# RohitMovva/VexAutonomousPlanner

Measured on NVIDIA B200. Metric: profiled trajectories/sec (8-node paths), higher is better.
Workload: dtype f64

## Files before the change

vexautonomousplanner_b200/csrc/vap_device.cuh:

```cuda
#pragma once
#include <cstdint>
#include <math.h>

#define NA 12
enum { A_X = 0, A_Y, A_TURN, A_WAIT, A_MAXVEL, A_MAXACC, A_TX, A_TY, A_INMAG, A_OUTMAG, A_RCOS, A_RSIN };
#define F_REVERSE 1
#define F_STOP 2
#define F_TANGENT 4
#define APA 4
enum { P_T = 0, P_WAIT, P_MAXVEL, P_MAXACC };

#define ST_OK 0
#define ST_FALSE (-1)
#define ST_INDEX (-2)
#define ST_VALUE (-3)
#define ST_CAPACITY (-4)
#define ST_DIVERGED (-5)
#define ST_EVENTS (-6)
#define VAP_ROW_LIMIT 50000000LL

#define VAP_PI 3.141592653589793

__device__ __forceinline__ void cp_async16(void* smem, const void* gmem)
{
    unsigned sa = (unsigned)__cvta_generic_to_shared(smem);
    asm volatile("cp.async.ca.shared.global [%0], [%1], 16;" ::"r"(sa), "l"(gmem));
}
__device__ __forceinline__ void cp_async_commit() { asm volatile("cp.async.commit_group;" ::); }
template <int N>
__device__ __forceinline__ void cp_async_wait() { asm volatile("cp.async.wait_group %0;" ::"n"(N) : "memory"); }

__device__ __forceinline__ void mbar_init(unsigned a, unsigned count)
{
    asm volatile("mbarrier.init.shared::cta.b64 [%0], %1;" ::"r"(a), "r"(count) : "memory");
}
__device__ __forceinline__ void mbar_expect_tx(unsigned a, unsigned bytes)
{
    asm volatile("mbarrier.arrive.expect_tx.shared::cta.b64 _, [%0], %1;" ::"r"(a), "r"(bytes) : "memory");
}
__device__ __forceinline__ void bulk_g2s(unsigned dst, const void* src, unsigned bytes, unsigned mbar)
{
    asm volatile("cp.async.bulk.shared::cluster.global.mbarrier::complete_tx::bytes [%0], [%1], %2, [%3];"
                 ::"r"(dst), "l"(src), "r"(bytes), "r"(mbar) : "memory");
}
__device__ __forceinline__ void mbar_wait(unsigned a, unsigned parity)
{
    asm volatile("{\n"
                 ".reg .pred P1;\n"
                 "LAB_WAIT:\n"
                 "mbarrier.try_wait.parity.shared::cta.b64 P1, [%0], %1;\n"
                 "@P1 bra DONE;\n"
                 "bra LAB_WAIT;\n"
                 "DONE:\n"
                 "}" ::"r"(a), "r"(parity) : "memory");
}

__device__ __forceinline__ void fence_mbar_init() { asm volatile("fence.mbarrier_init.release.cluster;" ::: "memory"); }
__device__ __forceinline__ void fence_proxy_async() { asm volatile("fence.proxy.async.shared::cta;" ::: "memory"); }

#ifdef VAP_BOUNDS_CHECK
#define VAP_DIAG_SITES 32
__device__ unsigned long long g_vap_diag[VAP_DIAG_SITES];
#define VAP_CHECK(site, cond) do { if (!(cond)) atomicAdd(&g_vap_diag[site], 1ull); else atomicAdd(&g_vap_diag[16 + ((site) & 15)], 1ull); } while (0)
#else
#define VAP_CHECK(site, cond) do { } while (0)
#endif

struct PathTile { long long b; unsigned x; };
__device__ __forceinline__ PathTile path_tile(unsigned tiles_x)
{
    PathTile p;
    const unsigned q = blockIdx.x / tiles_x;
    p.b = q; p.x = blockIdx.x - q * tiles_x;
    return p;
}

__device__ __forceinline__ double pymin(double a, double b) { return (b < a) ? b : a; }
__device__ __forceinline__ double pymax(double a, double b) { return (b > a) ? b : a; }
__device__ __forceinline__ double norm1d(double x, double y) { return sqrt(fma(y, y, x * x)); }
__device__ __forceinline__ double norm_ax1(double x, double y) { return sqrt(x * x + y * y); }
__device__ __forceinline__ double frac1(double t) { return t - floor(t); }
__device__ __forceinline__ double pymod_pos(double x, double y)
{
    double m = fmod(x, y);
    if (m != 0.0) { if (m < 0) m += y; } else m = 0.0;
    return m;
}

template <int WHICH>
__device__ __forceinline__ void basis(double t, double* H)
{
    double t2 = t * t, t3 = t2 * t;
    if (WHICH == 0) {
        double t4 = t3 * t, t5 = t4 * t;
        H[0] = 1 - 10 * t3 + 15 * t4 - 6 * t5;
        H[1] = 10 * t3 - 15 * t4 + 6 * t5;
        H[2] = t - 6 * t3 + 8 * t4 - 3 * t5;
        H[3] = -4 * t3 + 7 * t4 - 3 * t5;
        H[4] = 0.5 * t2 - 1.5 * t3 + 1.5 * t4 - 0.5 * t5;
        H[5] = 0.5 * t3 - t4 + 0.5 * t5;
    } else if (WHICH == 1) {
        double t4 = t3 * t;
        H[0] = -30 * t2 + 60 * t3 - 30 * t4;
        H[1] = 30 * t2 - 60 * t3 + 30 * t4;
        H[2] = 1 - 18 * t2 + 32 * t3 - 15 * t4;
        H[3] = -12 * t2 + 28 * t3 - 15 * t4;
        H[4] = t - 4.5 * t2 + 6 * t3 - 2.5 * t4;
        H[5] = 1.5 * t2 - 4 * t3 + 2.5 * t4;
    } else {
        H[0] = -60 * t + 180 * t2 - 120 * t3;
        H[1] = 60 * t - 180 * t2 + 120 * t3;
        H[2] = -36 * t + 96 * t2 - 60 * t3;
        H[3] = -24 * t + 84 * t2 - 60 * t3;
        H[4] = 1 - 9 * t + 18 * t2 - 10 * t3;
        H[5] = 3 * t - 12 * t2 + 10 * t3;
    }
}

__device__ __forceinline__ void normalize_param(double t, int nseg, double pend, int& idx, double& u)
{
    double tt = pymax(0.0, pymin(t, pend));
    idx = (int)tt;
    if (idx == nseg) idx = nseg - 1;
    u = tt - (double)idx;
}

template <int WHICH>
__device__ __forceinline__ void eval_spline(const double* __restrict__ seg, int nseg, double pend, double t,
                                            double& ox, double& oy)
{
    int idx; double u;
    normalize_param(t, nseg, pend, idx, u);
    double H[6];
    basis<WHICH>(u, H);
    const double2* s = reinterpret_cast<const double2*>(seg + (size_t)idx * 12);
    double ax = 0.0, ay = 0.0;
#pragma unroll
    for (int i = 0; i < 6; i++) { double2 r = __ldg(s + i); ax += H[i] * r.x; ay += H[i] * r.y; }
    ox = ax; oy = ay;
}

__device__ __forceinline__ void eval_spline_d12(const double* __restrict__ seg, int nseg, double pend, double t,
                                                double& dx, double& dy, double& ddx, double& ddy)
{
    int idx; double u;
    normalize_param(t, nseg, pend, idx, u);
    double H1[6], H2[6];
    basis<1>(u, H1);
    basis<2>(u, H2);
    const double2* s = reinterpret_cast<const double2*>(seg + (size_t)idx * 12);
    double ax = 0.0, ay = 0.0, bx = 0.0, by = 0.0;
#pragma unroll
    for (int i = 0; i < 6; i++) {
        double2 r = __ldg(s + i);
        ax += H1[i] * r.x; ay += H1[i] * r.y;
        bx += H2[i] * r.x; by += H2[i] * r.y;
    }
    dx = ax; dy = ay; ddx = bx; ddy = by;
}

struct PathGeo {
    const double* seg;
    const int* first;
    const double* pend;
    int S;
};
__device__ __forceinline__ int map_spline(const PathGeo& g, double t)
{
    int k = 0;
    if (g.S <= 8) {
        while (k < g.S - 1 && !(t <= (double)g.first[k + 1])) k++;
    } else {
        int lo = 0, hi = g.S - 1;
        while (lo < hi) {
            int mid = (lo + hi) >> 1;
            if (t <= (double)g.first[mid + 1]) hi = mid; else lo = mid + 1;
        }
        k = lo;
    }
    return k;
}
__device__ __forceinline__ PathGeo path_geo(long long b, int N_max, const double* seg, const int* first_node,
                                            const double* param_end, const int* n_splines)
{
    PathGeo g;
    g.seg = seg + (size_t)b * (N_max - 1) * 12;
    g.first = first_node + (size_t)b * (N_max + 1);
    g.pend = param_end + (size_t)b * N_max;
    g.S = n_splines[b];
    return g;
}

template <int WHICH>
__device__ __forceinline__ void eval_path(const PathGeo& g, double t, double& ox, double& oy)
{
    int k = map_spline(g, t);
    int f0 = g.first[k], f1 = g.first[k + 1];
    eval_spline<WHICH>(g.seg + (size_t)f0 * 12, f1 - f0, g.pend[k], t - (double)f0, ox, oy);
}
__device__ __forceinline__ void eval_path_d12(const PathGeo& g, double t, double& dx, double& dy, double& ddx,
                                              double& ddy)
{
    int k = map_spline(g, t);
    int f0 = g.first[k], f1 = g.first[k + 1];
    eval_spline_d12(g.seg + (size_t)f0 * 12, f1 - f0, g.pend[k], t - (double)f0, dx, dy, ddx, ddy);
}

__device__ __forceinline__ void curv_heading(double dx, double dy, double ddx, double ddy, double& kap, double& th)
{
    double s2 = dx * dx + dy * dy;
    double num = dx * ddy - dy * ddx;
    kap = (s2 >= 1e-10) ? num / (s2 * sqrt(s2)) : 0.0;
    th = atan2(dy, dx);
}

__device__ __forceinline__ double prop_param(long long j, long long P, int n, double step)
{
    return (j == P - 1) ? (double)(n - 1) : (double)j * step;
}
__device__ __forceinline__ long long prop_lower_bound(double t, long long P, int n, double step, double inv_step)
{
    double e = t * inv_step;
    long long j = (e > 0.0) ? (e < (double)P ? (long long)e : P) : 0;
    while (j > 0 && prop_param(j - 1, P, n, step) >= t) j--;
    while (j < P && prop_param(j, P, n, step) < t) j++;
    return j;
}
__device__ __forceinline__ double snap_gather(const double* __restrict__ vals, double t, long long P, int n,
                                              double step, double inv_step)
{
    long long idx = prop_lower_bound(t, P, n, step, inv_step);
    if (idx == 0) return vals[0];
    if (idx >= P) return vals[P - 1];
    double t0 = prop_param(idx - 1, P, n, step), t1 = prop_param(idx, P, n, step);
    if (frac1(t0) != frac1(t1)) return (frac1(t) > 0.5) ? vals[idx - 1] : vals[idx];
    double v0 = vals[idx - 1], v1 = vals[idx];
    return v0 + (v1 - v0) * (t - t0) / (t1 - t0);
}
__device__ __forceinline__ void snap_gather2(const double* __restrict__ ka, const double* __restrict__ ha, double t,
                                             long long P, int n, double step, double inv_step, double& k, double& h)
{
    long long idx = prop_lower_bound(t, P, n, step, inv_step);
    if (idx == 0) { k = ka[0]; h = ha[0]; return; }
    if (idx >= P) { k = ka[P - 1]; h = ha[P - 1]; return; }
    double t0 = prop_param(idx - 1, P, n, step), t1 = prop_param(idx, P, n, step);
    if (frac1(t0) != frac1(t1)) {
        long long g = (frac1(t) > 0.5) ? idx - 1 : idx;
        k = ka[g]; h = ha[g];
        return;
    }
    double w = (t - t0);
    k = ka[idx - 1] + (ka[idx] - ka[idx - 1]) * w / (t1 - t0);
    h = ha[idx - 1] + (ha[idx] - ha[idx - 1]) * w / (t1 - t0);
}

__device__ __forceinline__ double distance_to_time(const double* __restrict__ ld, const double* __restrict__ lt,
                                                   long long Q, double total, int n, double d, long long& hint)
{
    if (d <= 0) return 0.0;
    if (d >= total) return (double)(n - 1);
    long long idx;
    long long h = hint;
    if (h >= 1 && h < Q && ld[h - 1] < d) {
        idx = h;
        int steps = 0;
        while (idx < Q && ld[idx] < d && steps < 4) { idx++; steps++; }
        if (!(idx < Q && ld[idx] >= d)) h = -1;
    } else h = -1;
    if (h < 0) {
        long long lo = 0, hi = Q;
        while (lo < hi) {
            long long mid = lo + ((hi - lo) >> 1);
            if (ld[mid] < d) lo = mid + 1; else hi = mid;
        }
        idx = lo;
    }
    hint = idx;
    if (idx == 0) return lt[0];
    double d0 = ld[idx - 1], d1 = ld[idx], t0 = lt[idx - 1], t1 = lt[idx];
    return t0 + (t1 - t0) * (d - d0) / (d1 - d0);
}

struct PropGrid {
    int P, n;
    double step, inv_step;
};
__device__ __forceinline__ PropGrid prop_grid(int spn, int n)
{
    PropGrid g;
    g.P = spn * n; g.n = n;
    g.step = (double)(n - 1) / (double)(g.P - 1);
    g.inv_step = 1.0 / g.step;
    return g;
}
__device__ __forceinline__ double prop_param32(int j, const PropGrid& g)
{
    return (j == g.P - 1) ? (double)(g.n - 1) : (double)j * g.step;
}
__device__ __forceinline__ void snap_gather2_32(const double* __restrict__ ka, const double* __restrict__ ha, double t,
                                                const PropGrid& g, double& k, double& h)
{
    double e = t * g.inv_step;
    int j = (e > 0.0) ? (e < (double)g.P ? __double2int_rz(e) : g.P) : 0;
    while (j > 0 && prop_param32(j - 1, g) >= t) j--;
    while (j < g.P && prop_param32(j, g) < t) j++;
    if (j == 0) { k = ka[0]; h = ha[0]; return; }
    if (j >= g.P) { k = ka[g.P - 1]; h = ha[g.P - 1]; return; }
    double t0 = prop_param32(j - 1, g), t1 = prop_param32(j, g);
    if (frac1(t0) != frac1(t1)) {
        int q = (frac1(t) > 0.5) ? j - 1 : j;
        k = ka[q]; h = ha[q];
// ... 108 lines not shown
```

vexautonomousplanner_b200/csrc/vap_kernels.cu:

```cuda
#include <cuda_runtime.h>
#include <cstdio>
#include <cstring>
#include <cstdlib>

#include "../../include/vap.h"
#include "vap_device.cuh"
#include "vap_velocity.cuh"
#include "vap_timeloop.cuh"
#include "vap_format.cuh"

static thread_local char g_err[512] = "";
static int set_err(const char* where, cudaError_t e)
{
    snprintf(g_err, sizeof(g_err), "%s: %s", where, cudaGetErrorString(e));
    return -100;
}
static int arg_err(const char* msg)
{
    snprintf(g_err, sizeof(g_err), "%s", msg);
    return -101;
}
#define CHECK_LAUNCH(name)                                   \
    do {                                                     \
        cudaError_t e__ = cudaGetLastError();                \
// ... 187 lines not shown
        int m = i - cur + 1;
        RunView R;
        R.px = na + (size_t)cur * NA + A_X; R.py = na + (size_t)cur * NA + A_Y; R.stride = NA;
        R.has = nf + cur; R.has_stride = 1; R.in_mask = F_TANGENT; R.out_mask = F_TANGENT;
        R.tin = tin + 2 * cur; R.tout = tout + 2 * cur;
        fit_run(m, R, use_start, usx, usy, have_end, etx, ety, sg + (size_t)cur * 12, sl + cur, pr ? pr + pc : nullptr,
                pe + S, scr, use_start, have_end, nullptr, dv ? dv + (size_t)pc * 4 : nullptr);
        pc += m;
        S++;
        fn[S] = i;
        if ((rev || turn) && i < n - 1) cur = i;
    }
    n_splines[b] = (st == ST_OK) ? S : 0;
    status[b] = st;
}

__global__ void k_fit_splines(long long Rn, int n_max, const int* __restrict__ n_pts, const double* __restrict__ xy,
                              const int* __restrict__ tan_has, const double* __restrict__ tan_in,
                              const double* __restrict__ tan_out, const int* __restrict__ bnd_has,
                              const double* __restrict__ bnd, double* __restrict__ seg, double* __restrict__ seglen,
                              double* __restrict__ params, int* __restrict__ status, double* __restrict__ scratch,
                              const double* __restrict__ deriv_in, double* __restrict__ deriv_out)
{
    long long r = (long long)blockIdx.x * blockDim.x + threadIdx.x;
    if (r >= Rn) return;
    int n = n_pts[r];
    if (n < 2 || n > n_max) { status[r] = ST_FALSE; return; }
    RunView R;
    R.px = xy + (size_t)r * n_max * 2; R.py = R.px + 1; R.stride = 2;
    R.has = tan_has + (size_t)r * n_max; R.has_stride = 1; R.in_mask = 1; R.out_mask = 2;
    R.tin = tan_in + (size_t)r * n_max * 2; R.tout = tan_out + (size_t)r * n_max * 2;
    int bh = bnd_has[r];
    const double* bd = bnd + (size_t)r * 4;
    double pe;
    fit_run(n, R, (bh & 1) != 0, bd[0], bd[1], (bh & 2) != 0, bd[2], bd[3], seg + (size_t)r * (n_max - 1) * 12,
            seglen + (size_t)r * n_max, params + (size_t)r * n_max, &pe, scratch + (size_t)r * n_max * 5,
            (bh & 4) != 0, (bh & 8) != 0, (bh & 16) ? deriv_in + (size_t)r * n_max * 4 : nullptr,
            deriv_out ? deriv_out + (size_t)r * n_max * 4 : nullptr);
    status[r] = ST_OK;
}

__global__ void k_eval(long long n, const int* __restrict__ path, const double* __restrict__ t, int which, int N_max,
                       const double* __restrict__ seg, const int* __restrict__ first_node,
                       const double* __restrict__ param_end, const int* __restrict__ n_splines,
                       double* __restrict__ out)
{
    long long q = (long long)blockIdx.x * blockDim.x + threadIdx.x;
    if (q >= n) return;
    PathGeo g = path_geo(path[q], N_max, seg, first_node, param_end, n_splines);
    double ox = 0, oy = 0;
    if (g.S > 0) {
        if (which == 0) eval_path<0>(g, t[q], ox, oy);
        else if (which == 1) eval_path<1>(g, t[q], ox, oy);
        else if (which == 2) eval_path<2>(g, t[q], ox, oy);
        else {
            double dx, dy, ddx, ddy;
            eval_path_d12(g, t[q], dx, dy, ddx, ddy);
            double s2 = dx * dx + dy * dy;
            double den = s2 * sqrt(s2);
            ox = atan2(dy, dx);
            oy = (fabs(den) < 1e-10) ? 0.0 : (dx * ddy - dy * ddx) / den;
        }
    }
    out[2 * q] = ox; out[2 * q + 1] = oy;
}

__global__ void __launch_bounds__(256) k_build_lut(int N_max, const double* __restrict__ seg,
                                                   const int* __restrict__ first_node,
                                                   const double* __restrict__ param_end,
                                                   const int* __restrict__ n_splines, int* __restrict__ status,
                                                   int samples, long long Q_cap, double* __restrict__ lut_d,
                                                   double* __restrict__ lut_t, double* __restrict__ total_len)
{
    extern __shared__ double sm[];
    long long b = blockIdx.x;
    PathGeo g = path_geo(b, N_max, seg, first_node, param_end, n_splines);
    double* od = lut_d + (size_t)b * Q_cap;
    double* ot = lut_t + (size_t)b * Q_cap;
    const int st = status[b];
    const bool too_many = (long long)g.S * samples > Q_cap;
    if (st != ST_OK || g.S <= 0 || too_many) {
        __syncthreads();
        if (threadIdx.x == 0) {
            total_len[b] = 0.0;
            if (st == ST_OK && too_many) status[b] = ST_CAPACITY;
        }
        return;
    }
    double current = 0.0, prev_param = 0.0;
    for (int k = 0; k < g.S; k++) {
        int f0 = g.first[k], nseg = g.first[k + 1] - f0;
        double p1 = g.pend[k];
        const double* sg = g.seg + (size_t)f0 * 12;
        double step = (p1 - 0.0) / (double)(samples - 1);
        double lp1 = (samples > 2) ? 1.0 * step : p1;
        double dtp = lp1 - 0.0;
        for (int j = threadIdx.x; j < samples; j += blockDim.x) {
            double lp = (j == samples - 1) ? p1 : (double)j * step;
            double dx, dy;
            eval_spline<1>(sg, nseg, p1, lp, dx, dy);
            sm[j] = norm_ax1(dx, dy);
        }
        __syncthreads();
        double* inc = sm + samples;
        for (int j = threadIdx.x + 1; j < samples; j += blockDim.x) inc[j] = (sm[j - 1] + sm[j]) * 0.5 * dtp;
        __syncthreads();
        if (threadIdx.x == 0) {
            double c = 0.0;
            sm[0] = 0.0;
            int j = 1;
            for (; j + 8 <= samples; j += 8) {
                double a[8];
#pragma unroll
                for (int q = 0; q < 8; q++) a[q] = inc[j + q];
#pragma unroll
                for (int q = 0; q < 8; q++) { c = c + a[q]; sm[j + q] = c; }
            }
            for (; j < samples; j++) { c = c + inc[j]; sm[j] = c; }
        }
        __syncthreads();
        for (int j = threadIdx.x; j < samples; j += blockDim.x) {
            double lp = (j == samples - 1) ? p1 : (double)j * step;
            od[(size_t)k * samples + j] = sm[j] + current;
            ot[(size_t)k * samples + j] = lp + prev_param;
        }
        current = sm[samples - 1] + current;
        prev_param += p1 - 0.0;
        __syncthreads();
    }
    if (threadIdx.x == 0) total_len[b] = current;
}

__global__ void __launch_bounds__(256) k_build_lut_index(const int* __restrict__ n_splines, const int* __restrict__ status,
                                                         int samples, long long Q_cap, const double* __restrict__ lut_d,
                                                         const double* __restrict__ total_len, int* __restrict__ lut_inv)
{
    const long long b = blockIdx.x;
    int* row = lut_inv + (size_t)b * (Q_cap + LUT_INV_HDR + 2);
    const int S = n_splines[b];
    if (status[b] != ST_OK || S <= 0 || (long long)S * samples > Q_cap) return;
    const int Q = S * samples;
    const double* ld = lut_d + (size_t)b * Q_cap;
    const double L = total_len[b];
    const double scale = (L > 0.0) ? (double)Q / L : 0.0;
    if (threadIdx.x == 0) { row[0] = __double2loint(scale); row[1] = __double2hiint(scale); }
    for (int m = threadIdx.x; m <= Q; m += blockDim.x) {
        const double x = (scale > 0.0) ? (double)m / scale : 0.0;
        int lo = 0, hi = Q;
        while (lo < hi) { int mid = (lo + hi) >> 1; if (ld[mid] < x) lo = mid + 1; else hi = mid; }
        row[LUT_INV_HDR + m] = lo > Q - 1 ? Q - 1 : lo;
    }
}

#ifndef PROPS_PER_THREAD
#define PROPS_PER_THREAD 8
#endif
__global__ void __launch_bounds__(256) k_build_props(int N_max, const int* __restrict__ n_nodes,
                                                     const double* __restrict__ seg,
                                                     const int* __restrict__ first_node,
                                                     const double* __restrict__ param_end,
                                                     const int* __restrict__ n_splines,
                                                     const int* __restrict__ status, int spn, long long P_cap,
                                                     double* __restrict__ prop_k, double* __restrict__ prop_h,
                                                     unsigned tiles_x)
{
    const PathTile pt = path_tile(tiles_x);
    const long long b = pt.b;
    const int n = n_nodes[b];
    const int P = spn * n;
    int j = (int)pt.x * (blockDim.x * PROPS_PER_THREAD) + threadIdx.x;
    if (status[b] != ST_OK || j >= P || (long long)P > P_cap) return;
    const PathGeo g = path_geo(b, N_max, seg, first_node, param_end, n_splines);
    const double step = (double)(n - 1) / (double)(P - 1);
    double* pk = prop_k + (size_t)b * P_cap;
    double* ph = prop_h + (size_t)b * P_cap;
#pragma unroll 1
    for (int it = 0; it < PROPS_PER_THREAD && j < P; ++it, j += blockDim.x) {
        const double t = prop_param(j, P, n, step);
        double dx, dy, ddx, ddy, k, h;
        eval_path_d12(g, t, dx, dy, ddx, ddy);
        curv_heading(dx, dy, ddx, ddy, k, h);
        pk[j] = k;
        ph[j] = h;
    }
}

__global__ void k_query_tables(long long n, const int* __restrict__ path, const double* __restrict__ x, int what,
                               const int* __restrict__ n_nodes, const int* __restrict__ n_splines, int samples,
                               long long Q_cap, const double* __restrict__ lut_d, const double* __restrict__ lut_t,
                               const double* __restrict__ total_len, int spn, long long P_cap,
                               const double* __restrict__ prop_k, const double* __restrict__ prop_h,
                               double* __restrict__ out)
{
    long long q = (long long)blockIdx.x * blockDim.x + threadIdx.x;
    if (q >= n) return;
    long long b = path[q];
    int nn = n_nodes[b];
    if (what == 0) {
        long long hint = -1;
        out[q] = distance_to_time(lut_d + (size_t)b * Q_cap, lut_t + (size_t)b * Q_cap, (long long)samples * n_splines[b],
                                  total_len[b], nn, x[q], hint);
    } else {
        long long P = (long long)spn * nn;
        double step = (double)(nn - 1) / (double)(P - 1);
        const double* v = (what == 1 ? prop_h : prop_k) + (size_t)b * P_cap;
        out[q] = snap_gather(v, x[q], P, nn, step, 1.0 / step);
    }
}

__global__ void k_build_dgrid(long long n, double dd, double* __restrict__ dgrid)
{
    if (blockIdx.x != 0 || threadIdx.x != 0) return;
    double d = 0.0;
    for (long long i = 0; i < n; i++) { dgrid[i] = d; d += dd; }
}

__global__ void k_count_samples(long long B, const int* __restrict__ status_in, int* __restrict__ status,
                                long long n_grid, const double* __restrict__ dgrid,
                                const double* __restrict__ total_len, long long D_cap, int* __restrict__ n_samples)
{
    long long b = (long long)blockIdx.x * blockDim.x + threadIdx.x;
    if (b >= B) return;
    if (status_in[b] != ST_OK) { n_samples[b] = 0; return; }
    double L = total_len[b];
    long long lo = 0, hi = n_grid;
    while (lo < hi) {
        long long mid = lo + ((hi - lo) >> 1);
        if (dgrid[mid] < L) lo = mid + 1; else hi = mid;
    }
    long long D = lo + 1;
    if (lo >= n_grid) {
        const double est = ceil(L / (dgrid[1] - dgrid[0])) + 2.0;
        D = est < 2147483647.0 ? (long long)est : 2147483647LL;
        if (D <= D_cap) D = D_cap + 1;
    }
    if (lo >= n_grid || D > D_cap) { status[b] = ST_CAPACITY; n_samples[b] = (int)(D > 2147483647LL ? 2147483647LL : D); return; }
    n_samples[b] = (int)D;
}

__global__ void __launch_bounds__(256) k_dist_sample(const int* __restrict__ n_nodes,
                                                     const int* __restrict__ n_splines,
                                                     const int* __restrict__ status, const double* __restrict__ dgrid,
                                                     int samples, long long Q_cap, const double* __restrict__ lut_d,
                                                     const double* __restrict__ lut_t,
                                                     const double* __restrict__ total_len, int spn, long long P_cap,
                                                     const double* __restrict__ prop_k,
                                                     const double* __restrict__ prop_h, long long D_cap,
                                                     const int* __restrict__ n_samples, double* __restrict__ t_out,
                                                     double* __restrict__ kap, double* __restrict__ th, unsigned tiles_x)
{
    const PathTile pt = path_tile(tiles_x);
    long long b = pt.b;
    long long i = (long long)pt.x * blockDim.x + threadIdx.x;
    if (status[b] != ST_OK) return;
    long long D = n_samples[b];
    if (i >= D) return;
    int n = n_nodes[b];
    double t;
    if (i == D - 1) t = (double)(n - 1);
    else {
        long long hint = -1;
        t = distance_to_time(lut_d + (size_t)b * Q_cap, lut_t + (size_t)b * Q_cap, (long long)samples * n_splines[b],
                             total_len[b], n, dgrid[i], hint);
    }
    long long P = (long long)spn * n;
    double step = (double)(n - 1) / (double)(P - 1);
    double k, h;
    snap_gather2(prop_k + (size_t)b * P_cap, prop_h + (size_t)b * P_cap, t, P, n, step, 1.0 / step, k, h);
    size_t o = (size_t)b * D_cap + i;
    t_out[o] = t; kap[o] = k; th[o] = h;
}

__global__ void __launch_bounds__(64) k_fwd_bwd(long long B, int N_max, int A_max, const double* __restrict__ node_attr,
                                                const int* __restrict__ node_flags, const int* __restrict__ n_nodes,
                                                const double* __restrict__ ap_attr, const int* __restrict__ ap_flags,
                                                const int* __restrict__ n_ap, const double* __restrict__ cons,
                                                const int* __restrict__ status, double dd, double dt, double start_vel,
                                                double end_vel, long long D_cap, const int* __restrict__ n_samples,
                                                const double* __restrict__ tq, const double* __restrict__ kap,
                                                const double* __restrict__ th, double* __restrict__ vel, int E_cap,
                                                double* __restrict__ max_accels, int* __restrict__ bidx,
                                                int* __restrict__ bval, int* __restrict__ n_ev,
                                                double* __restrict__ t_est, int mode)
{
    long long b = (long long)blockIdx.x * blockDim.x + threadIdx.x;
    if (b >= B) return;
    if (status[b] != ST_OK) { n_ev[2 * b] = 0; n_ev[2 * b + 1] = 0; if (t_est) t_est[b] = 0.0; return; }
    const int n = n_nodes[b];
    const int A = n_ap ? n_ap[b] : 0;
    const double* na = node_attr + (size_t)b * N_max * NA;
    const int* nf = node_flags + (size_t)b * N_max;
    const double* apa = ap_attr + (size_t)b * A_max * APA;
    const int* apf = ap_flags + (size_t)b * A_max;
    const double V = cons[b * 6 + 0], A0 = cons[b * 6 + 1], w = cons[b * 6 + 5];
    const long long D = n_samples[b];
    const double* T = tq + (size_t)b * D_cap;
    const double* K = kap + (size_t)b * D_cap;
    const double* H = th + (size_t)b * D_cap;
    double* vv = vel + (size_t)b * D_cap;
    double* ma = max_accels + (size_t)b * E_cap;
    int* bi = bidx + (size_t)b * E_cap;
    int* bv = bval + (size_t)b * E_cap;

    const double max_angular_vel = 2 * V / w;
    const double max_angular_accel = 2 * A0 / w;
    const double t_end = (double)(n - 1);

    int node_num = 0, action_idx = 0, n_acc = 0, n_b = 0;
    double max_velocity = (na[A_MAXVEL] > 0) ? na[A_MAXVEL] : V;
    ma[n_acc++] = (na[A_MAXACC] > 0) ? na[A_MAXACC] : A0;
    bi[0] = 0; bv[0] = 0; n_b = 1;

    double acc = A0, dec = cons[b * 6 + 2];
    int bptr = 0;
    double prev_ang_vel = 0.0;
    double v_i = start_vel;
    vv[0] = start_vel;
    double t_i = T[0], th_i = H[0];
    for (long long i = 0; i < D - 1; i++) {
        double v0n, t_n = T[i + 1], th_n = H[i + 1];
        if (i + 1 < D - 1) {
            v0n = max_velocity;
            if (frac1(t_i) > frac1(t_n) && t_n < t_end) {
                node_num += 1;
                const double* a = na + (size_t)node_num * NA;
                if (nf[node_num] & F_STOP) v0n = 0.01;
                max_velocity = (a[A_MAXVEL] > 0) ? a[A_MAXVEL] : V;
                ma[n_acc++] = (a[A_MAXACC] > 0) ? a[A_MAXACC] : A0;
                if (node_num < n - 1) {
                    if (bi[n_b - 1] == (int)(i + 1)) bv[n_b - 1] = n_acc - 1;
                    else { bi[n_b] = (int)(i + 1); bv[n_b] = n_acc - 1; n_b++; }
                }
            }
            if (action_idx < A && t_i < apa[action_idx * APA + P_T] && t_n >= apa[action_idx * APA + P_T]) {
                const double* p = apa + (size_t)action_idx * APA;
                max_velocity = (p[P_MAXVEL] > 0) ? p[P_MAXVEL] : V;
// ... 304 lines not shown
    const double* sg = seg + ((size_t)b * (N_max - 1) + f0) * 12;
    if (mode == 0) {
        double t0 = a[q], t1 = bb[q];
        if (t0 >= t1 || t0 < 0.0 || t1 > pend) { qstatus[q] = ST_VALUE; out[q] = 0.0; return; }
        out[q] = gl_arclen(sg, nseg, pend, t0, t1, npts, pts, wts);
        qstatus[q] = ST_OK;
    } else {
        double s = a[q], tol = bb[q];
        if (s < 0) { qstatus[q] = ST_VALUE; out[q] = 0.0; return; }
        double total = gl_arclen(sg, nseg, pend, 0.0, pend, npts, pts, wts);
        if (s > total) { qstatus[q] = ST_VALUE; out[q] = 0.0; return; }
        qstatus[q] = ST_OK;
        if (s == 0) { out[q] = 0.0; return; }
        if (s == total) { out[q] = pend; return; }
        double lo = 0.0, hi = pend;
        for (int it = 0; it < max_iter; it++) {
            double m = (lo + hi) / 2;
            double len = gl_arclen(sg, nseg, pend, 0.0, m, npts, pts, wts);
            double err = len - s;
            if (fabs(err) < tol) { out[q] = m; return; }
            if (err > 0) hi = m; else lo = m;
        }
        out[q] = (lo + hi) / 2;
    }
}

__global__ void k_turn_profile(long long n, const double* __restrict__ q, int mode, long long K_cap,
                               double* __restrict__ out_a, double* __restrict__ out_b, int* __restrict__ counts)
{
    long long i = (long long)blockIdx.x * blockDim.x + threadIdx.x;
    if (i >= n) return;
    const double* p = q + (size_t)i * 5;
    double x = p[0], V = p[1], A = p[2], w = p[3], dt = p[4];
    double* oa = out_a + (size_t)i * K_cap;
    if (mode == 1) {
        Trapezoid tz = trapezoid_setup(V, A, x, dt);
        counts[i] = (int)tz.K;
        for (long long j = 0; j < tz.K && j < K_cap; j++) oa[j] = trapezoid_vel(tz, j, dt);
        return;
    }
    double* ob = out_b + (size_t)i * K_cap;
    Trapezoid tz = trapezoid_setup(V, A, fabs(x) * w / 2, dt);
    counts[i] = (int)tz.K;
    double sgn = x > 0 ? -1.0 : 1.0, accum = 0.0, hprev = 0.0;
    for (long long j = 0; j < tz.K && j < K_cap; j++) {
        double v = trapezoid_vel(tz, j, dt);
        double h = (accum / (w / 2)) * sgn;
        accum += v * dt;
        oa[j] = h;
        ob[j] = (j == 0) ? 0.0 : (h - hprev) / dt;
        hprev = h;
    }
}

__global__ void k_lerp(long long n, const double* __restrict__ x, long long m, const double* __restrict__ xs,
                       const double* __restrict__ ys, double* __restrict__ out)
{
    long long i = (long long)blockIdx.x * blockDim.x + threadIdx.x;
    if (i >= n) return;
    double xv = x[i];
    long long lo = 0, hi = m;
    while (lo < hi) {
        long long mid = lo + ((hi - lo) >> 1);
        if (xs[mid] <= xv) lo = mid + 1; else hi = mid;
    }
    long long idx = lo - 1;
    if (idx < 0) { out[i] = ys[0]; return; }
    if (idx >= m - 1) { out[i] = ys[m - 1]; return; }
    double x0 = xs[idx], x1 = xs[idx + 1], y0 = ys[idx], y1 = ys[idx + 1];
    out[i] = y0 + (xv - x0) * (y1 - y0) / (x1 - x0);
}

__global__ void k_wheel(long long n, const double* __restrict__ lin, const double* __restrict__ ang, double tw,
                        double* __restrict__ left, double* __restrict__ right)
{
    long long i = (long long)blockIdx.x * blockDim.x + threadIdx.x;
    if (i >= n) return;
    double l = lin[i], a = ang[i];
    left[i] = l - (a * tw / 2);
    right[i] = l + (a * tw / 2);
}

static inline unsigned blocks_for(long long n, int bs) { return (unsigned)((n + bs - 1) / bs); }
#define STREAM ((cudaStream_t)stream)

extern "C" int vap_build_path(int64_t B, int N_max, const double* node_attr, const int32_t* node_flags,
                              const int32_t* n_nodes, double* seg, int32_t* first_node, double* param_end,
                              double* seglen, int32_t* n_splines, int32_t* status, double* scratch, double* params,
                              double* derivs, void* stream)
{
    if (B <= 0) return 0;
    if (N_max < 2) return arg_err("vap_build_path: N_max < 2");
    k_build_path<<<blocks_for(B, 128), 128, 0, STREAM>>>(B, N_max, node_attr, node_flags, n_nodes, seg, first_node,
                                                        param_end, seglen, n_splines, status, scratch, params, derivs);
    CHECK_LAUNCH("vap_build_path");
    return 0;
}

extern "C" int vap_fit_splines(int64_t R, int n_max, const int32_t* n_pts, const double* xy, const int32_t* tan_has,
                               const double* tan_in, const double* tan_out, const int32_t* bnd_has, const double* bnd,
                               double* seg, double* seglen, double* params, int32_t* status, double* scratch,
                               const double* deriv_in, double* deriv_out, void* stream)
{
    if (R <= 0) return 0;
    if (n_max < 2) return arg_err("vap_fit_splines: n_max < 2");
    k_fit_splines<<<blocks_for(R, 128), 128, 0, STREAM>>>(R, n_max, n_pts, xy, tan_has, tan_in, tan_out, bnd_has, bnd,
                                                         seg, seglen, params, status, scratch, deriv_in, deriv_out);
    CHECK_LAUNCH("vap_fit_splines");
    return 0;
}

extern "C" int vap_eval(int64_t n, const int32_t* path, const double* t, int which, int N_max, const double* seg,
                        const int32_t* first_node, const double* param_end, const int32_t* n_splines, double* out,
                        void* stream)
{
    if (n <= 0) return 0;
    if (which < 0 || which > 3) return arg_err("vap_eval: which must be 0..3");
    k_eval<<<blocks_for(n, 128), 128, 0, STREAM>>>(n, path, t, which, N_max, seg, first_node, param_end, n_splines, out);
    CHECK_LAUNCH("vap_eval");
    return 0;
}

extern "C" int vap_build_lut(int64_t B, int N_max, const double* seg, const int32_t* first_node,
                             const double* param_end, const int32_t* n_splines, int32_t* status, int samples,
                             int64_t Q_cap, double* lut_d, double* lut_t, double* total_len, void* stream)
{
    if (B <= 0) return 0;
    if (samples < 2 || samples > 6000) return arg_err("vap_build_lut: samples must be in [2, 6000]");
    const size_t lut_sm = 2 * (size_t)samples * sizeof(double);
    if (lut_sm > 48 * 1024) cudaFuncSetAttribute(k_build_lut, cudaFuncAttributeMaxDynamicSharedMemorySize, (int)lut_sm);
    k_build_lut<<<(unsigned)B, 256, lut_sm, STREAM>>>(N_max, seg, first_node, param_end,
                                                                               n_splines, status, samples, Q_cap,
                                                                               lut_d, lut_t, total_len);
    CHECK_LAUNCH("vap_build_lut");
    return 0;
}

extern "C" int64_t vap_lut_index_row_ints(int64_t Q_cap) { return Q_cap + LUT_INV_HDR + 2; }
extern "C" int vap_build_lut_index(int64_t B, const int32_t* n_splines, const int32_t* status, int samples, int64_t Q_cap,
                                   const double* lut_d, const double* total_len, int32_t* lut_inv, void* stream)
{
    if (B <= 0) return 0;
    k_build_lut_index<<<(unsigned)B, 256, 0, STREAM>>>(n_splines, status, samples, Q_cap, lut_d, total_len, lut_inv);
    CHECK_LAUNCH("vap_build_lut_index");
    return 0;
}

extern "C" int vap_build_props(int64_t B, int N_max, const int32_t* n_nodes, const double* seg,
                               const int32_t* first_node, const double* param_end, const int32_t* n_splines,
                               const int32_t* status, int spn, int64_t P_cap, double* prop_k, double* prop_h,
                               void* stream)
{
    if (B <= 0) return 0;
    const unsigned tx = blocks_for(P_cap, 256 * PROPS_PER_THREAD);
    if ((long long)tx * B > 2147483647LL) return arg_err("vap_build_props: more than 2^31 CTAs (tile the batch)");
    const unsigned grid = tx * (unsigned)B;
    k_build_props<<<grid, 256, 0, STREAM>>>(N_max, n_nodes, seg, first_node, param_end, n_splines, status, spn, P_cap,
                                            prop_k, prop_h, tx);
    CHECK_LAUNCH("vap_build_props");
    return 0;
}

extern "C" int vap_query_tables(int64_t n, const int32_t* path, const double* x, int what, const int32_t* n_nodes,
                                const int32_t* n_splines, int samples, int64_t Q_cap, const double* lut_d,
                                const double* lut_t, const double* total_len, int spn, int64_t P_cap,
                                const double* prop_k, const double* prop_h, double* out, void* stream)
{
    if (n <= 0) return 0;
    k_query_tables<<<blocks_for(n, 128), 128, 0, STREAM>>>(n, path, x, what, n_nodes, n_splines, samples, Q_cap, lut_d,
                                                          lut_t, total_len, spn, P_cap, prop_k, prop_h, out);
    CHECK_LAUNCH("vap_query_tables");
    return 0;
}

extern "C" int vap_build_dgrid(int64_t n, double dd, double* dgrid, void* stream)
{
    if (n <= 0) return 0;
    k_build_dgrid<<<1, 1, 0, STREAM>>>(n, dd, dgrid);
    CHECK_LAUNCH("vap_build_dgrid");
    return 0;
}

extern "C" int vap_build_lerp_recip(int64_t n, double dd, double* rden, void* stream)
{
    if (n <= 0) return 0;
    k_build_lerp_recip<<<blocks_for(n, 256), 256, 0, STREAM>>>(n, dd, rden);
    CHECK_LAUNCH("vap_build_lerp_recip");
    return 0;
}

extern "C" int vap_dist_sample(int64_t B, const int32_t* n_nodes, const int32_t* n_splines, int32_t* status,
                               int64_t n_grid, const double* dgrid, int samples, int64_t Q_cap, const double* lut_d,
                               const double* lut_t, const double* total_len, int spn, int64_t P_cap,
                               const double* prop_k, const double* prop_h, int64_t D_cap, int32_t* n_samples,
                               double* t, double* kap, double* th, void* stream)
{
    if (B <= 0) return 0;
    k_count_samples<<<blocks_for(B, 128), 128, 0, STREAM>>>(B, status, status, n_grid, dgrid, total_len, D_cap, n_samples);
    CHECK_LAUNCH("vap_dist_sample/count");
    const unsigned tx = blocks_for(D_cap, 256);
    if ((long long)tx * B > 2147483647LL) return arg_err("vap_dist_sample: more than 2^31 CTAs (tile the batch)");
    const unsigned grid = tx * (unsigned)B;
    k_dist_sample<<<grid, 256, 0, STREAM>>>(n_nodes, n_splines, status, dgrid, samples, Q_cap, lut_d, lut_t, total_len,
                                            spn, P_cap, prop_k, prop_h, D_cap, n_samples, t, kap, th, tx);
    CHECK_LAUNCH("vap_dist_sample");
    return 0;
}

extern "C" int vap_fwd_bwd(int64_t B, int N_max, int A_max, const double* node_attr, const int32_t* node_flags,
                           const int32_t* n_nodes, const double* ap_attr, const int32_t* ap_flags, const int32_t* n_ap,
                           const double* cons, const int32_t* status, double dd, double dt, double start_vel,
                           double end_vel, int64_t D_cap, const int32_t* n_samples, const double* t, const double* kap,
                           const double* th, double* vel, int E_cap, double* max_accels, int32_t* bidx, int32_t* bval,
                           int32_t* n_ev, double* t_est, int mode, void* stream)
{
    if (B <= 0) return 0;
    if (E_cap < N_max + A_max + 2) return arg_err("vap_fwd_bwd: E_cap < N_max + A_max + 2");
    k_fwd_bwd<<<blocks_for(B, 32), 32, 0, STREAM>>>(B, N_max, A_max, node_attr, node_flags, n_nodes, ap_attr, ap_flags,
                                                   n_ap, cons, status, dd, dt, start_vel, end_vel, D_cap, n_samples, t,
                                                   kap, th, vel, E_cap, max_accels, bidx, bval, n_ev, t_est, mode);
    CHECK_LAUNCH("vap_fwd_bwd");
    return 0;
}

extern "C" int vap_resample(int64_t B, int N_max, int A_max, const double* node_attr, const int32_t* node_flags,
                            const int32_t* n_nodes, const double* ap_attr, const int32_t* ap_flags, const int32_t* n_ap,
                            const double* cons, int32_t* status, double dt, double dd, const double* seg,
                            const int32_t* first_node, const double* param_end, const int32_t* n_splines, int samples,
                            int64_t Q_cap, const double* lut_d, const double* lut_t, const double* total_len, int spn,
                            int64_t P_cap, const double* prop_k, const double* prop_h, int64_t D_cap,
                            const int32_t* n_samples, const double* vel, int64_t T_cap, double* out,
                            int32_t* nodes_map, int32_t* actions_map, int32_t* n_maps, int32_t* n_out, double* summary,
                            void* stream)
{
    if (B <= 0) return 0;
    k_resample<<<blocks_for(B, 32), 32, 0, STREAM>>>(B, N_max, A_max, node_attr, node_flags, n_nodes, ap_attr, ap_flags,
                                                    n_ap, cons, status, dt, dd, seg, first_node, param_end, n_splines,
                                                    samples, Q_cap, lut_d, lut_t, total_len, spn, P_cap, prop_k, prop_h,
                                                    D_cap, n_samples, vel, T_cap, out, nodes_map, actions_map, n_maps,
                                                    n_out, summary, 0, 0);
    CHECK_LAUNCH("vap_resample");
    return 0;
}

extern "C" int vap_gl(int64_t n, const int32_t* path, const int32_t* spl, const double* a, const double* b, int mode,
                      int max_iter, int npts, const double* gl_pts, const double* gl_wts, int N_max, const double* seg,
                      const int32_t* first_node, const double* param_end, double* out, int32_t* qstatus, void* stream)
{
    if (n <= 0) return 0;
    if (npts < 1 || npts > 128) return arg_err("vap_gl: npts must be in [1, 128]");
    k_gl<<<blocks_for(n, 64), 64, 0, STREAM>>>(n, path, spl, a, b, mode, max_iter, npts, gl_pts, gl_wts, N_max, seg,
                                              first_node, param_end, out, qstatus);
    CHECK_LAUNCH("vap_gl");
    return 0;
}

extern "C" int vap_turn_profile(int64_t n, const double* q, int mode, int64_t K_cap, double* out_a, double* out_b,
                                int32_t* counts, void* stream)
{
    if (n <= 0) return 0;
    k_turn_profile<<<blocks_for(n, 64), 64, 0, STREAM>>>(n, q, mode, K_cap, out_a, out_b, counts);
    CHECK_LAUNCH("vap_turn_profile");
    return 0;
}

extern "C" int vap_lerp(int64_t n, const double* x, int64_t m, const double* xs, const double* ys, double* out,
                        void* stream)
{
    if (n <= 0) return 0;
    if (m < 1) return arg_err("vap_lerp: empty table");
    k_lerp<<<blocks_for(n, 128), 128, 0, STREAM>>>(n, x, m, xs, ys, out);
    CHECK_LAUNCH("vap_lerp");
    return 0;
}

extern "C" int vap_wheel_trajectory(int64_t n, const double* lin, const double* ang, double track_width, double* left,
                                    double* right, void* stream)
{
    if (n <= 0) return 0;
    k_wheel<<<blocks_for(n, 256), 256, 0, STREAM>>>(n, lin, ang, track_width, left, right);
    CHECK_LAUNCH("vap_wheel_trajectory");
    return 0;
}

extern "C" int64_t vap_event_scratch_ints(int64_t B, int N_max, int A_max)
{
    int Am = A_max > 0 ? A_max : 1;
    return B * N_max + B + B * Am * EV_AP_CAND + B * Am;
}

struct EventScratch { int32_t *wrap, *nwrap, *apc, *napc; };
static cudaError_t event_scratch(int32_t* ev_scratch, int64_t B, int N_max, int Am, cudaStream_t st, EventScratch& c)
{
    c.wrap = ev_scratch;
    c.nwrap = c.wrap + (size_t)B * N_max;
    c.apc = c.nwrap + B;
    c.napc = c.apc + (size_t)B * Am * EV_AP_CAND;
    cudaError_t e = cudaMemsetAsync(c.nwrap, 0, sizeof(int32_t) * (size_t)B, st);
    if (e != cudaSuccess) return e;
    return cudaMemsetAsync(c.napc, 0, sizeof(int32_t) * (size_t)B * Am, st);
}

extern "C" int64_t vap_pass_row_slots(int64_t D_cap, int chunks) { return ((D_cap + 8 * (int64_t)chunks + 64 + 1) / 2) * 2; }

template <int NT>
static int launch_passes(int64_t B, size_t ss, cudaStream_t st, const double* cons, const int32_t* status, double dd, double dt,
                         double start_vel, double end_vel, long long RS, long long D_cap, const int32_t* n_samples,
                         const double* rec, int E_cap, const double* max_accels, const int32_t* bidx, const int32_t* bval,
                         const int32_t* n_ev, const int32_t* vr_idx, const double* vr_val, const int32_t* st_idx,
                         const int32_t* n_vr, double* vel_f, double* vel, float* t_est, int32_t* rounds, bool backward,
// ... 631 lines not shown
```

Measured before the change: 1.263 million.

## Group paths per thread in props kernel and reuse spline basis across paths

The property-building kernel now assigns each thread one sample index j across a group of 16 paths, instead of several indices within a single path. Paths with the same node count map j to the same parameter u, so the Hermite basis weights are recomputed only when u changes, and the step division is reused as well. This targets the wasted CTAs and repeated basis arithmetic when paths are short (8 nodes). In exchange, each thread loops serially over 16 paths and the grid shrinks, which may lower the available parallelism.

New measurement: 1.259 million, median of 6. About the same (-0.3%).

```diff
diff --git a/vexautonomousplanner_b200/csrc/vap_device.cuh b/vexautonomousplanner_b200/csrc/vap_device.cuh
--- a/vexautonomousplanner_b200/csrc/vap_device.cuh
+++ b/vexautonomousplanner_b200/csrc/vap_device.cuh
@@ -140,15 +140,10 @@
     ox = ax; oy = ay;
 }
 
-__device__ __forceinline__ void eval_spline_d12(const double* __restrict__ seg, int nseg, double pend, double t,
-                                                double& dx, double& dy, double& ddx, double& ddy)
-{
-    int idx; double u;
-    normalize_param(t, nseg, pend, idx, u);
-    double H1[6], H2[6];
-    basis<1>(u, H1);
-    basis<2>(u, H2);
-    const double2* s = reinterpret_cast<const double2*>(seg + (size_t)idx * 12);
+__device__ __forceinline__ void segment_d12(const double* __restrict__ seg_row, const double* H1, const double* H2,
+                                            double& dx, double& dy, double& ddx, double& ddy)
+{
+    const double2* s = reinterpret_cast<const double2*>(seg_row);
     double ax = 0.0, ay = 0.0, bx = 0.0, by = 0.0;
 #pragma unroll
     for (int i = 0; i < 6; i++) {
@@ -157,6 +152,16 @@
         bx += H2[i] * r.x; by += H2[i] * r.y;
     }
     dx = ax; dy = ay; ddx = bx; ddy = by;
+}
+__device__ __forceinline__ void eval_spline_d12(const double* __restrict__ seg, int nseg, double pend, double t,
+                                                double& dx, double& dy, double& ddx, double& ddy)
+{
+    int idx; double u;
+    normalize_param(t, nseg, pend, idx, u);
+    double H1[6], H2[6];
+    basis<1>(u, H1);
+    basis<2>(u, H2);
+    segment_d12(seg + (size_t)idx * 12, H1, H2, dx, dy, ddx, ddy);
 }
 
 struct PathGeo {
diff --git a/vexautonomousplanner_b200/csrc/vap_kernels.cu b/vexautonomousplanner_b200/csrc/vap_kernels.cu
--- a/vexautonomousplanner_b200/csrc/vap_kernels.cu
+++ b/vexautonomousplanner_b200/csrc/vap_kernels.cu
@@ -363,10 +363,10 @@
     }
 }
 
-#ifndef PROPS_PER_THREAD
-#define PROPS_PER_THREAD 8
+#ifndef PROPS_GROUP
+#define PROPS_GROUP 16
 #endif
-__global__ void __launch_bounds__(256) k_build_props(int N_max, const int* __restrict__ n_nodes,
+__global__ void __launch_bounds__(256) k_build_props(long long B, int N_max, const int* __restrict__ n_nodes,
                                                      const double* __restrict__ seg,
                                                      const int* __restrict__ first_node,
                                                      const double* __restrict__ param_end,
@@ -376,23 +376,35 @@
                                                      unsigned tiles_x)
 {
     const PathTile pt = path_tile(tiles_x);
-    const long long b = pt.b;
-    const int n = n_nodes[b];
-    const int P = spn * n;
-    int j = (int)pt.x * (blockDim.x * PROPS_PER_THREAD) + threadIdx.x;
-    if (status[b] != ST_OK || j >= P || (long long)P > P_cap) return;
-    const PathGeo g = path_geo(b, N_max, seg, first_node, param_end, n_splines);
-    const double step = (double)(n - 1) / (double)(P - 1);
-    double* pk = prop_k + (size_t)b * P_cap;
-    double* ph = prop_h + (size_t)b * P_cap;
+    const int j = (int)pt.x * blockDim.x + threadIdx.x;
+    const long long b0 = pt.b * PROPS_GROUP;
+    const long long b1 = (b0 + PROPS_GROUP < B) ? b0 + PROPS_GROUP : B;
+    int n_step = -1;
+    double step = 0.0;
+    unsigned long long u_bits = ~0ull;
+    double H1[6], H2[6];
 #pragma unroll 1
-    for (int it = 0; it < PROPS_PER_THREAD && j < P; ++it, j += blockDim.x) {
+    for (long long b = b0; b < b1; ++b) {
+        const int n = n_nodes[b];
+        const int P = spn * n;
+        if (status[b] != ST_OK || j >= P || (long long)P > P_cap) continue;
+        if (n != n_step) { step = (double)(n - 1) / (double)(P - 1); n_step = n; }
         const double t = prop_param(j, P, n, step);
-        double dx, dy, ddx, ddy, k, h;
-        eval_path_d12(g, t, dx, dy, ddx, ddy);
-        curv_heading(dx, dy, ddx, ddy, k, h);
-        pk[j] = k;
-        ph[j] = h;
+        const PathGeo g = path_geo(b, N_max, seg, first_node, param_end, n_splines);
+        const int k = map_spline(g, t);
+        const int f0 = g.first[k], f1 = g.first[k + 1];
+        int idx; double u;
+        normalize_param(t - (double)f0, f1 - f0, g.pend[k], idx, u);
+        if ((unsigned long long)__double_as_longlong(u) != u_bits) {
+            basis<1>(u, H1);
+            basis<2>(u, H2);
+            u_bits = (unsigned long long)__double_as_longlong(u);
+        }
+        double dx, dy, ddx, ddy, kap, h;
+        segment_d12(g.seg + (size_t)(f0 + idx) * 12, H1, H2, dx, dy, ddx, ddy);
+        curv_heading(dx, dy, ddx, ddy, kap, h);
+        prop_k[(size_t)b * P_cap + j] = kap;
+        prop_h[(size_t)b * P_cap + j] = h;
     }
 }
 
@@ -1003,10 +1015,11 @@
                                void* stream)
 {
     if (B <= 0) return 0;
-    const unsigned tx = blocks_for(P_cap, 256 * PROPS_PER_THREAD);
-    if ((long long)tx * B > 2147483647LL) return arg_err("vap_build_props: more than 2^31 CTAs (tile the batch)");
-    const unsigned grid = tx * (unsigned)B;
-    k_build_props<<<grid, 256, 0, STREAM>>>(N_max, n_nodes, seg, first_node, param_end, n_splines, status, spn, P_cap,
+    const unsigned tx = blocks_for(P_cap, 256);
+    const long long groups = (B + PROPS_GROUP - 1) / PROPS_GROUP;
+    if ((long long)tx * groups > 2147483647LL) return arg_err("vap_build_props: more than 2^31 CTAs (tile the batch)");
+    const unsigned grid = tx * (unsigned)groups;
+    k_build_props<<<grid, 256, 0, STREAM>>>(B, N_max, n_nodes, seg, first_node, param_end, n_splines, status, spn, P_cap,
                                             prop_k, prop_h, tx);
     CHECK_LAUNCH("vap_build_props");
     return 0;
```
